# ajparra/iRotAvg

Measured on AMD Instinct MI355X. Metric: IRLS edge-updates/sec (+ iters-to-converge), higher is better.
Workload: dtype f64

## Files before the change

### irotavg_amd/capi.py

```python
import ctypes as C
import os

import numpy as np

_HERE = os.path.dirname(os.path.abspath(__file__))
LIB_PATH = os.path.join(_HERE, "libirotavg_hip.so")

OK = 0
ERR_BAD_ARG, ERR_NOT_SPANNING, ERR_SOLVER, ERR_UNKNOWN_COST = -1, -2, -3, -4
ERR_NOMEM, ERR_HIP, ERR_NO_DEVICE, ERR_NOT_CONVERGED = -5, -6, -7, -8
ERR_UNSUPPORTED = -9

SYMBOLS = [
    "irotavg_default_options", "irotavg_init_mst", "irotavg_make_A", "irotavg_l1ra", "irotavg_irls",
    "irotavg_quat_normalised", "irotavg_graph_create", "irotavg_graph_destroy",
    "irotavg_graph_set_rotations", "irotavg_graph_get_rotations",
    "irotavg_graph_snapshot_rotations", "irotavg_graph_restore_rotations", "irotavg_graph_get_weights",
    "irotavg_graph_set_weights", "irotavg_graph_irls", "irotavg_graph_l1ra",
    "irotavg_graph_quat_normalised", "irotavg_graph_get_stats", "irotavg_graph_reset_stats",
    "irotavg_graph_synchronize", "irotavg_graph_edge_residual", "irotavg_graph_get_residuals",
    "irotavg_graph_ls_solve", "irotavg_graph_update_weights", "irotavg_graph_apply_step",
    "irotavg_graph_l1decode_pd", "irotavg_graph_time_kernel", "irotavg_graph_fingerprint", "irotavg_version",
    "irotavg_device_count", "irotavg_error_string",
    "irotavg_viewgraph_create", "irotavg_viewgraph_destroy", "irotavg_viewgraph_add_view",
# ... 366 lines not shown
        return r

    def ls_solve(self, allow_rc=(), return_rc=False):
        X = np.zeros((self.nu, 3), order="F")
        rc = lib().irotavg_graph_ls_solve(self._h, _d(X), self.nu)
        if rc != OK and rc not in allow_rc:
            raise IrotavgError(rc, "irotavg_graph_ls_solve")
        return (rc, X) if return_rc else X

    def update_weights(self, cost, sigma):
        check(lib().irotavg_graph_update_weights(self._h, cost, sigma), "update_weights")

    def apply_step(self):
        s = C.c_double(0)
        check(lib().irotavg_graph_apply_step(self._h, C.byref(s)), "apply_step")
        return s.value

    def l1decode_pd(self, y, pdmaxiter=2):
        y = np.ascontiguousarray(y, dtype=np.float64)
        assert y.shape == (self.m,)
        x = np.zeros(self.nu)
        stuck = C.c_int(0)
        check(lib().irotavg_graph_l1decode_pd(self._h, _d(y), pdmaxiter, _d(x), C.byref(stuck)),
              "l1decode_pd")
        return x, stuck.value

    def direct_info(self):
        out = (C.c_int64 * 64)()
        k = lib().irotavg_graph_direct_info(self._h, out, 64)
        if k < 0:
            raise IrotavgError(k, "direct_info")
        if out[0] == 0:
            return dict(block=0, levels=[], closures=0, fused_assembly=0, unit_factor=0, unit_factor_solves=0,
                        unit_factor_bytes=0)
        nl = int(out[1])
        return dict(block=int(out[0]), levels=[dict(blocks=int(out[2 + 3 * l]), chunks=int(out[3 + 3 * l]),
                                                    reduced=int(out[4 + 3 * l])) for l in range(nl)],
                    closures=int(out[2 + 3 * nl]), fused_assembly=int(out[3 + 3 * nl]) if k > 3 + 3 * nl else 0,
                    unit_factor=int(out[4 + 3 * nl]) if k > 4 + 3 * nl else 0,
                    unit_factor_solves=int(out[5 + 3 * nl]) if k > 5 + 3 * nl else 0,
                    unit_factor_bytes=int(out[6 + 3 * nl]) if k > 6 + 3 * nl else 0)

    def direct_residual(self):
        out = np.zeros(3)
        check(lib().irotavg_graph_direct_residual(self._h, _d(out)), "direct_residual")
        return out

    def rotation_variance(self, pairs=None, marginals=True, allow_rc=()):
        return _variance_call(lambda *a: lib().irotavg_graph_rotation_variance(self._h, *a), self.n_total, pairs,
                              marginals, allow_rc, "irotavg_graph_rotation_variance")

    def edge_diagnostics(self, edge_var=True, leverage=True, chi2=True, allow_rc=()):
        return _edge_call(lambda *a: lib().irotavg_graph_edge_diagnostics(self._h, *a), self.m, edge_var, leverage,
                          chi2, allow_rc, "irotavg_graph_edge_diagnostics")

    def pose_weights(self, cost, sigma):
        check(lib().irotavg_graph_pose_weights(self._h, int(cost), float(sigma)), "irotavg_graph_pose_weights")

    def fingerprint(self):
        out = (C.c_uint64 * 512)()
        n = lib().irotavg_graph_fingerprint(self._h, out, 512)
        if n < 0:
            raise IrotavgError(n, "fingerprint")
        return [int(out[i]) for i in range(n)]

    FINGERPRINT_TAIL = ("l0_far_entries", "asm_windowed", "asm_l1_fused", "l1_fused", "cg2", "ndense", "ndense_pad",
                        "dense_bw", "mg_dense_max", "mg_kc_x1000", "additive_top")

    def fingerprint_scalars(self):
        fp = self.fingerprint()
        k = len(self.FINGERPRINT_TAIL)
        if not k <= len(fp) < 512:
            raise ValueError("fingerprint truncated: %d words" % len(fp))
        return dict(zip(self.FINGERPRINT_TAIL, fp[-k:]))
# ... 378 lines not shown
```

### irotavg_amd/csrc/bcr.hip

```cpp
#include <atomic>

#include "graph.hpp"
#include "kernels.hpp"
#include "asm0w.hpp"

namespace irh {
constexpr double kBcrGateTolMin = 1e-12;

typedef double v4d __attribute__((ext_vector_type(4)));
typedef double v2d __attribute__((ext_vector_type(2)));
typedef int v2i __attribute__((ext_vector_type(2)));

constexpr int kTopMax = 16, kTopRounds = 6;
struct BcrTopSched {
    int n = 0, nr = 0, last = 0;
    signed char ne[kTopRounds];
    signed char i[kTopRounds][4], a[kTopRounds][4], c[kTopRounds][4];
};

#if defined(__HIP_DEVICE_COMPILE__)
#define IRH_GPTR(T) T __attribute__((address_space(1))) *
#else
#define IRH_GPTR(T) T *
#endif
// ... 1632 lines not shown
        if (NR > 3)
            for (int q = 0; q < nfar; q++) Z[(size_t)row * zstride + zoff + q] = xs[3 + q];
        if (NR == 3 && Qap) acc_ap += step_apply(xs[0], xs[1], xs[2], Qap, row + fap, true);
    };
    if (L0) {
        const int row0 = chunk * 8 * B;
        for (int t = tid; t < kreal * B; t += 256) {
            const int row = row0 + t, blk = t / B;
            if (row < n) put_row(row, bcr_pos(placed, kreal, blk) * B + (t - blk * B));
        }
    } else {
        for (int e = tid; e < 8 * B * NR; e += 256) {
            const int blk = e / (B * NR);
            xl[(size_t)chunk * 8 * B * NR + e] =
                blk < kreal ? (&sX[1][0])[bcr_pos(placed, kreal, blk) * B * NR + (e - blk * B * NR)] : 0.0;
        }
        if (chunk * 8 + 8 > nred && nred < nb)
            for (int t = tid; t < 8 * B; t += 256) {
                const int i = t / B, r = t - i * B, gb = chunk * 8 + i;
                if (gb >= nred && gb < nb) {
                    const int row = (8 * nred + (gb - nred)) * B + r;
                    if (row < n) put_row(row, t);
                }
            }
    }
    if (NR == 3 && Qap) bcr_apply_sum(acc_ap, part_ap, slot0 + chunk);
}

struct BcrBackPlan {
    const double *W[kMaxLevels];
    int nb[kMaxLevels];
    int top, base;
};
constexpr int kBackTopThreads = 512;
template <int B>
__global__ __launch_bounds__(kBackTopThreads) void k_bcr_back_top(BcrBackPlan P, const double *__restrict__ xtop, double *__restrict__ xl,
                                                       double4 *__restrict__ X, int n, int nred,
                                                       double4 *__restrict__ Qap = nullptr, int fap = 0,
                                                       double *__restrict__ part_ap = nullptr, int slot0 = 0,
                                                       int top_all = 0) {
    constexpr int NR = 3;
    typedef BcrDim<B, NR> Dm;
    constexpr int WB = B * Dm::NC, XB = B * NR;
    constexpr int NV = (7 * WB / 2 + kBackTopThreads - 1) / kBackTopThreads;
    __shared__ double sW[7 * WB];
    __shared__ double sX[9][XB];
    __shared__ double sWin[2][16][XB];
    const int tid = threadIdx.x, lane = tid & 63;
    const int wave = __builtin_amdgcn_readfirstlane(tid >> 6);
    const int cbase = blockIdx.x;
    auto range = [&](int L, int &lo, int &hi) {
        lo = hi = cbase;
        for (int l = P.base; l < L; l++) {
            lo = (lo > 0 ? lo - 1 : 0) >> 3;
            hi >>= 3;
        }
    };
    auto wanted = [&](int L, int q) {
        if (L == P.base) return 0x7f;
        int lo, hi, m = 0;
        range(L - 1, lo, hi);
        for (int j = (lo > 0 ? lo - 1 : 0); j <= hi; j++)
            if ((j >> 3) == q && (j & 7) < 7) m |= 1 << (j & 7);
        return bcr_back_mask(m);
    };
    v2d wreg[NV];
    auto request = [&](int L, int q) {
        const int kreal = P.nb[L] - q * 8 < 8 ? P.nb[L] - q * 8 : 8;
        const int nblk = kreal > 7 ? 7 : kreal;
        const int mask = wanted(L, q);
        const v2d *__restrict__ src = reinterpret_cast<const v2d *>(P.W[L] + (size_t)q * 7 * WB);
#pragma unroll
        for (int v = 0; v < NV; v++) {
            const int e = tid + kBackTopThreads * v, blk = e / (WB / 2);
            wreg[v] = (blk < nblk && ((mask >> blk) & 1)) ? __builtin_nontemporal_load(&src[e]) : v2d{0.0, 0.0};
        }
    };
    auto deposit = [&]() {
        v2d *dst = reinterpret_cast<v2d *>(sW);
#pragma unroll
        for (int v = 0; v < NV; v++) {
            const int e = tid + kBackTopThreads * v;
            if (e < 7 * WB / 2) dst[e] = wreg[v];
        }
    };
    double acc_ap = 0.0;
    int L = P.top, lo, hi;
    range(L, lo, hi);
    int q = lo;
    request(L, q);
    while (true) {
        int plo = 0, phi = 0;
        if (L < P.top) range(L + 1, plo, phi);
        const double(*winP)[XB] = sWin[(L + 1) & 1];
        double(*winC)[XB] = sWin[L & 1];
        const int kreal = P.nb[L] - q * 8 < 8 ? P.nb[L] - q * 8 : 8;
        const int mask = wanted(L, q);
        deposit();
        for (int e = tid; e < 7 * XB; e += kBackTopThreads) (&sX[1][0])[e] = 0.0;
        for (int e = tid; e < XB; e += kBackTopThreads) {
            sX[8][e] = L == P.top ? xtop[(top_all ? q * XB : 0) + e] : winP[q - 8 * plo][e];
            sX[0][e] = q == 0 ? 0.0 : L == P.top ? (top_all ? xtop[(q - 1) * XB + e] : 0.0) : winP[q - 1 - 8 * plo][e];
        }
        int Ln = L, qn = q + 1;
        if (qn > hi) {
            Ln = L - 1;
            if (Ln >= P.base) {
                range(Ln, lo, hi);
                qn = lo;
            }
        }
        if (Ln >= P.base) request(Ln, qn);
        __syncthreads();
        bcr_back_rounds<B, NR, kBackTopThreads / 64>(sW, sX, false, kreal, wave, lane, mask);
        if (L > P.base) {
            int clo, chi;
            range(L, clo, chi);
            for (int e = tid; e < 8 * XB; e += kBackTopThreads) {
                const int blk = e / XB;
                winC[(q - clo) * 8 + blk][e - blk * XB] = blk < kreal ? (&sX[1][0])[e] : 0.0;
            }
        } else {
            for (int e = tid; e < 8 * XB; e += kBackTopThreads) {
                const int blk = e / XB;
                xl[(size_t)q * 8 * XB + e] = blk < kreal ? (&sX[1][0])[e] : 0.0;
            }
            if (q * 8 + 8 > nred && nred < P.nb[L])
                for (int t = tid; t < 8 * B; t += kBackTopThreads) {
                    const int i = t / B, r = t - i * B, gb = q * 8 + i;
                    if (gb >= nred && gb < P.nb[L]) {
                        const int row = (8 * nred + (gb - nred)) * B + r;
                        const double *xs = &sX[1][0] + t * NR;
                        if (row < n) {
                            X[row] = double4{xs[0], xs[1], xs[2], 0.0};
                            if (Qap) acc_ap += step_apply(xs[0], xs[1], xs[2], Qap, row + fap, true);
                        }
                    }
                }
        }
        if (Ln < P.base) break;
        __syncthreads();
        L = Ln;
        q = qn;
    }
    if (Qap) bcr_apply_sum(acc_ap, part_ap, slot0 + cbase);
}

struct BcrClPlan {
    const double *W[kMaxLevels], *Dinv[kMaxLevels];
    double *Wrw[kMaxLevels];
    const double *topDinv;
    double *xtop;
};

template <int B, int NWF = 4>
__global__ __launch_bounds__(64 * NWF) void k_bcr_closure_forward(BcrClPlan P, int r, int nslots, const int *__restrict__ off,
                                                              const int4 *__restrict__ steps,
                                                              const int4 *__restrict__ init, double *__restrict__ recR,
                                                              double *__restrict__ recW, double *__restrict__ T,
                                                              const double *__restrict__ slot_init = nullptr,
                                                              const int2 *__restrict__ fin = nullptr,
                                                              const int *__restrict__ gid = nullptr,
                                                              double *__restrict__ dep = nullptr, int world = 0,
                                                              int rank = 0) {
    constexpr int NR = 3, NC = 2 * B + NR, BB = B * B, NCOL = NC + B, NE = B * NCOL;
    constexpr int NLD = (NE + 63) / 64;
    constexpr int KP = B == 24 ? 3 : (NCOL * 4 <= 256 ? 4 : 2), KB = B / KP;
    static_assert(B % KP == 0 && NCOL * KP <= 256, "thread (col, part)");
    extern __shared__ double smem[];
    const int lane = threadIdx.x & 63, wave = __builtin_amdgcn_readfirstlane(threadIdx.x >> 6);
    const int q = blockIdx.x;
    double *stage = smem + (size_t)wave * NE;
    double *spart = smem + (size_t)NWF * NE;
    double *slots = spart + KP * NCOL;
    if (wave == 0) {
        if (slot_init) {
            for (int e = lane; e < nslots * B; e += 64) slots[e] = slot_init[(size_t)q * nslots * B + e];
        } else {
// ... 747 lines not shown
        if (l > 0) L.x.alloc((size_t)L.nch * 8 * B * NR);
        if (nb <= 8 && !g.bcr_shard) {
            S.top16 = false;
            break;
        }
        L.sepD.alloc((size_t)L.nch * B * B);
        L.extD.alloc((size_t)L.nch * B * B);
        L.extG.alloc((size_t)L.nch * B * B);
        L.sepR.alloc((size_t)L.nch * B * NR);
        L.extR.alloc((size_t)L.nch * B * NR);
        if (nb <= 8) break;
        nb = L.nch + (l == 0 ? nraw : 0);
        nch = (nb + 7) / 8;
    }
    if (g.bcr_shard) {
        S.ext0 = g.bcr_ext0;
        S.ghost_extcol.upload(g.bcr_ghost_extcol, g.stream);
        S.remD.alloc((size_t)B * B);
        S.remR.alloc((size_t)B * NR);
        IRH_CHECK(hipStreamSynchronize(g.stream));
    }
    S.xtop.alloc((size_t)B * NR);
    if (S.nfar > 0) bcr_closure_plan(g);
    if (g.bcr_shard && !g.bcr_fix_row.empty()) {
        S.nfix = (int)g.bcr_fix_row.size();
        S.fix_row.upload(g.bcr_fix_row, g.stream);
        S.fix_off.upload(g.bcr_fix_off, g.stream);
        S.fix_e.upload(g.bcr_fix_e, g.stream);
        S.fix_saved.alloc((size_t)S.nfix);
        IRH_CHECK(hipStreamSynchronize(g.stream));
    }
}

template <int B, int NR>
static void bcr_run(Graph &g, int only, int pass, bool open_top = false, int phase = 0, const double *xc_top = nullptr,
                    const double *xext = nullptr) {
    BcrState &S = *g.bcr;
    Level &L0 = g.levels[0];
    hipStream_t st = g.stream;
    const int nl = (int)S.lev.size();
    const int dbg = S.dbg_word >= 0 ? S.dbg_word : g.sw.bcr_dbg;
    long long *stamps = nullptr;
    if (dbg & 64) {
        if (!S.stamps.p) S.stamps.alloc((size_t)S.lev[0].nch * 16);
        stamps = S.stamps.p;
    }
    const int nfar = 0;
    const int *fi = nullptr, *fj = nullptr;
    (void)pass;
    bool fused_up = false;
    if constexpr (NR == 3 && B <= 24) {
        fused_up = nl >= 3 && nl - 1 <= kUpLevels && only < 0 && phase == 0 && !open_top && !g.bcr_shard && S.nfar == 0 &&
                   S.lev[1].nch <= 256 && !(dbg & 64) && !g.bcr_no_fused_up;
        if ((dbg & 128) && !S.stamps.p) S.stamps.alloc((size_t)std::max(S.lev[0].nch * 16, 32 * kUpLevels));
        if (fused_up) fused_up = bcr_up_reserve<B>(g, S.lev[1].nch);
    }
    if (only < 0 && phase != 2) S.up_used = false;
    int uf = 0;
    BcrUnit &U = S.unit;
    if (only < 0 && phase != 2) U.last = 0;
    if constexpr (NR == 3 && (B == 8 || B == 16 || B == 24)) {
        const int req = g.bcr_unit_req;
        if (req && fused_up && S.top16 && dbg == 0 && !g.bcr_guard && !g.bcr_out && !g.sw.bcr_no_unit_factor &&
            (g.bcr_asm_fused || req == 3)) {
            if (!U.lev.empty() && U.epoch != g_unit_epoch.load(std::memory_order_acquire)) U.release();
            uf = U.valid ? 2 : (req == 1 ? 1 : 0);
// ... 167 lines not shown
                }
#undef IRH_BCR_LAUNCH_ASM
            }
        }
        if (asm0) continue;
#define IRH_BCR_LAUNCH(L0_, TOP_)                                                                                   \
    if constexpr (B <= 24) {                                                                                        \
        if (wide)                                                                                                   \
            hipLaunchKernelGGL((k_bcr_reduce<B, NR, L0_, TOP_, 8>), dim3(L.nch), dim3(512), 0, st, IRH_BCR_ARGS);   \
        else                                                                                                        \
            hipLaunchKernelGGL((k_bcr_reduce<B, NR, L0_, TOP_, 4>), dim3(L.nch), dim3(256), 0, st, IRH_BCR_ARGS);   \
    } else {                                                                                                        \
        hipLaunchKernelGGL((k_bcr_reduce<B, NR, L0_, TOP_, 4>), dim3(L.nch), dim3(256), 0, st, IRH_BCR_ARGS);       \
    }
        if (l == 0 && top) {
            IRH_BCR_LAUNCH(true, true)
        } else if (l == 0) {
            IRH_BCR_LAUNCH(true, false)
        } else if (top) {
            IRH_BCR_LAUNCH(false, true)
        } else {
            IRH_BCR_LAUNCH(false, false)
        }
#undef IRH_BCR_LAUNCH
#undef IRH_BCR_ARGS
    }
    double4 *Xout = g.bcr_out ? g.bcr_out : g.X.p + g.ng;
    bool fused_back = false;
    const int ltop = S.top16 ? nl - 2 : nl - 1;
    if constexpr (NR == 3) fused_back = ltop >= 1 && !g.bcr_shard && !open_top;
    const bool apply = NR == 3 && g.bcr_apply && only < 0 && phase == 0 && (fused_back || (S.top16 && nl == 2)) && !g.bcr_out &&
                       g.ng == 0;
    g.bcr_applied = apply;
    for (int l = ltop; l >= 0 && phase != 1 && !uf_up_only; l--) {
        if (only >= 0 && only != 100 + l) continue;
        BcrLevel &L = S.lev[l];
        if constexpr (NR == 3) {
            if (fused_back && l >= 1) {
                if (l > 1) continue;
                BcrBackPlan P;
                for (int k = 0; k < nl; k++) {
                    P.W[k] = uf && k + 1 < nl ? U.lev[(size_t)k].Wu.p : S.lev[k].W.p;
                    P.nb[k] = S.lev[k].nb;
                }
                P.top = ltop;
                P.base = 1;
                hipLaunchKernelGGL((k_bcr_back_top<B>), dim3(L.nch), dim3(kBackTopThreads), 0, st, P,
                                   S.top16 ? S.lev[nl - 1].x.p : S.xtop.p, L.x.p, Xout, L0.n, L.nred,
                                   apply ? g.Q.p : (double4 *)nullptr, g.f, g.part_score.p, S.lev[0].nch, (int)S.top16);
                continue;
            }
        }
        const double *xc = l == nl - 1 ? (open_top ? xc_top : S.xtop.p) : S.lev[l + 1].x.p;
        if (l == 0)
            hipLaunchKernelGGL((k_bcr_back<B, NR, true>), dim3(L.nch), dim3(256), 0, st, L.nb, L.nred, L0.n,
                               uf ? U.lev[0].Wu.p : L.W.p, xc,
                               (double *)nullptr, Xout, (double *)nullptr, 0, 0, nfar, xext, (int)g.bcr_shard,
                               apply ? g.Q.p : (double4 *)nullptr, g.f, g.part_score.p, 0);
        else
            hipLaunchKernelGGL((k_bcr_back<B, NR, false>), dim3(L.nch), dim3(256), 0, st, L.nb, L.nred, L0.n, L.W.p, xc,
                               L.x.p, Xout, (double *)nullptr, 0, 0, nfar, xext, (int)g.bcr_shard);
    }
}

template <int B>
static void bcr_launch_forward(hipStream_t st, const BcrClPlan &P, int r, int nslots, const int *off, const int4 *steps,
                               const int4 *init, double *recR, double *recW, double *T, const double *slot_init,
                               const int2 *fin, const int *gid, double *dep, int world, int rank);

template <int B>
static void bcr_run_all(Graph &g, int only) {
    BcrState &S = *g.bcr;
    if (S.nfar == 0 || only >= 0) {
        bcr_run<B, 3>(g, only, 0);
        return;
    }
    hipStream_t st = g.stream;
    const int r = S.nfar, npad = S.cl_npad, nl = (int)S.lev.size();
    if (!S.dead_clean) IRH_CHECK(hipMemsetAsync(S.dead.p, 0, sizeof(int), st));
// ... 361 lines not shown
    T.co_elim.upload(elim, st);
    T.xbuf.alloc(T.x_doubles());
    T.Dinv.alloc((size_t)7 * B * B);
    T.topDinv.alloc((size_t)B * B);
    T.recR.alloc((size_t)r * nst * B);
    T.recW.alloc((size_t)r * nst * B);
    T.Ttop.alloc((size_t)r * 3);
    T.lam.alloc((size_t)T.npad * 3);
    T.dead.alloc(1);
    IRH_CHECK(hipMemsetAsync(T.topDinv.p, 0, sizeof(double) * (size_t)B * B, st));
    IRH_CHECK(hipMemsetAsync(T.xbuf.p, 0, sizeof(double) * T.x_doubles(), st));
    IRH_CHECK(hipStreamSynchronize(st));
}
#define IRH_BCR_DISPATCH(fn, ...)              \
    switch (g.bcr_B) {                         \
    case 8: fn<8>(__VA_ARGS__); break;         \
    case 16: fn<16>(__VA_ARGS__); break;       \
    case 24: fn<24>(__VA_ARGS__); break;       \
    default: fn<32>(__VA_ARGS__); break;       \
    }
void bcr_shard_reduce(Graph &g, BcrTop &T, int rank) {
    bcr_alloc(g);
    IRH_BCR_DISPATCH(bcr_shard_reduce_t, g, T, rank)
}
void bcr_top_solve(Graph &g, BcrTop &T) { IRH_BCR_DISPATCH(bcr_top_solve_t, g, T) }
void bcr_shard_back(Graph &g, BcrTop &T, int rank) {
    IRH_BCR_DISPATCH(bcr_shard_back_t, g, T, rank)
    g.stats.direct_solves += 1;
}
void bcr_shard_closures_forward(Graph &g, BcrTop &T, int rank) { IRH_BCR_DISPATCH(bcr_shard_closures_forward_t, g, T, rank) }
void bcr_top_solve_closures(Graph &g, BcrTop &T) { IRH_BCR_DISPATCH(bcr_top_solve_closures_t, g, T) }
void bcr_shard_closures_correct(Graph &g, BcrTop &T) { IRH_BCR_DISPATCH(bcr_shard_closures_correct_t, g, T) }

int bcr_solve(Graph &g, int only) {
    if (!g.bcr_B) return IROTAVG_ERR_BAD_ARG;
    bcr_alloc(g);
    switch (g.bcr_B) {
    case 8: bcr_run_all<8>(g, only); break;
    case 12: bcr_run_all<12>(g, only); break;
    case 16: bcr_run_all<16>(g, only); break;
    case 20: bcr_run_all<20>(g, only); break;
    case 24: bcr_run_all<24>(g, only); break;
    case 28: bcr_run_all<28>(g, only); break;
    case 32: bcr_run_all<32>(g, only); break;
    default: return IROTAVG_ERR_BAD_ARG;
    }
    if (only < 0) g.stats.direct_solves += 1;
    return IROTAVG_OK;
}

__global__ __launch_bounds__(256) void k_bcr_residual(int n, const int *__restrict__ sl_off, const int *__restrict__ col,
                                                       const double *__restrict__ val, const double *__restrict__ diag,
                                                       const double4 *__restrict__ rhs, const double4 *__restrict__ X,
                                                       double *__restrict__ part) {
    const int row = blockIdx.x * 256 + threadIdx.x;
    double r0 = 0.0, r1 = 0.0, r2 = 0.0, b0 = 0.0, b1 = 0.0, b2 = 0.0;
    if (row < n) {
        const int sl = row >> 6, ln = row & 63;
        const int o0 = sl_off[sl], w = sl_off[sl + 1] - o0;
        const v2i *__restrict__ cp = reinterpret_cast<const v2i *>(col) + (size_t)(o0 / 2) * 64 + ln;
        const v2d *__restrict__ vp = reinterpret_cast<const v2d *>(val) + (size_t)(o0 / 2) * 64 + ln;
        const double4 x = X[row], bb = rhs[row];
        const double d = diag[row];
        double s0 = d * x.x, s1 = d * x.y, s2 = d * x.z;
        for (int q = 0; q < w / 2; q++) {
            const v2i cc = cp[(size_t)q * 64];
// ... 42 lines not shown
    double rr[3] = {0, 0, 0}, bb[3] = {0, 0, 0};
    for (int b = 0; b < grid; b++)
        for (int c = 0; c < 3; c++) {
            rr[c] += h[(size_t)b * 8 + c];
            bb[c] += h[(size_t)b * 8 + 4 + c];
        }
    for (int c = 0; c < 3; c++) {
        relres[c] = bb[c] > 0.0 ? std::sqrt(rr[c] / bb[c]) : (rr[c] > 0.0 ? HUGE_VAL : 0.0);
        g.stats.last_relres[c] = relres[c];
    }
    return IROTAVG_OK;
}

int bcr_info(Graph &g, int64_t *out, int cap) {
    int k = 0;
    auto put = [&](int64_t v) {
        if (k < cap) out[k++] = v;
    };
    put(g.bcr_B);
    if (!g.bcr_B) return k;
    bcr_alloc(g);
    put((int64_t)g.bcr->lev.size());
    for (const BcrLevel &L : g.bcr->lev) {
        put(L.nb);
        put(L.nch);
        put(L.nred);
    }
    put(g.bcr->nfar);
    put(g.bcr_asm_fused_last ? 1 : 0);
    const bool stored = bcr_unit_valid(g);
    put(stored ? 1 : 0);
    put(g.bcr->unit.solves);
    put(stored ? g.bcr->unit.bytes : 0);
    return k;
}

int bcr_stamps_up(Graph &g, double *out) {
    if (!g.bcr_B) return IROTAVG_ERR_BAD_ARG;
    bcr_alloc(g);
    BcrState &S = *g.bcr;
    struct DbgScope {
        BcrState &S;
        ~DbgScope() { S.dbg_word = -1; }
    } dbg_scope{S};
    S.dbg_word = 128 + 256 * g.sw.bcr_stamp_chunk;
    const size_t cnt = (size_t)std::max(S.lev[0].nch * 16, 32 * kUpLevels);
    if (!S.stamps.p) S.stamps.alloc(cnt);
    IRH_CHECK(hipMemsetAsync(S.stamps.p, 0, sizeof(long long) * cnt, g.stream));
    const int rc = bcr_solve(g, -1);
    S.dbg_word = -1;
    if (rc != IROTAVG_OK) return rc;
    long long h[32 * kUpLevels];
    IRH_CHECK(hipMemcpyAsync(h, S.stamps.p, sizeof(h), hipMemcpyDeviceToHost, g.stream));
    IRH_CHECK(hipStreamSynchronize(g.stream));
    bcr_up_release(g);
    for (int k = 0; k < 32 * kUpLevels; k++) out[k] = !h[k] ? -1.0 : (k & 31) >= 20 ? (double)h[k] : (double)(h[k] - h[16]);
    return S.up_used ? IROTAVG_OK : IROTAVG_ERR_BAD_ARG;
}

int bcr_stamps(Graph &g, int level, int chunk, double *out) {
    if (!g.bcr_B) return IROTAVG_ERR_BAD_ARG;
    bcr_alloc(g);
    BcrState &S = *g.bcr;
    if (level < 0 || level >= (int)S.lev.size() || chunk < 0 || chunk >= S.lev[level].nch) return IROTAVG_ERR_BAD_ARG;
    struct DbgScope {
        BcrState &S;
// ... 562 lines not shown
```

### irotavg_amd/csrc/graph.hpp

```cpp
#pragma once
#include <functional>
#include <memory>

#include "common.hpp"
#include "hostwait.hpp"

namespace irh {

struct Graph;
void bcr_up_release(Graph &g) noexcept;
struct BcrState;
struct BcrDeleter {
    void operator()(BcrState *p) const;
};

struct Graph {
    int64_t m = 0, n_total = 0, mpad = 0;
    int f = 0, nu = 0, ng = 0, no = 0;
    irotavg_options opt{};
    Switches sw;
    hipStream_t stream = nullptr;
    int device = 0;

    DevBuf<int> ei, ej;
// ... 59 lines not shown

    DevBuf<double> pd;
    DevBuf<double> pdn;
    DevBuf<double> pd_part;
    bool pd_ready = false;
    const double *pd_rhs_src = nullptr;
    bool pd_rhs_done = false;
    std::vector<std::unique_ptr<Graph>> l1_clones;
    bool is_clone = false;

    double *hpin = nullptr;
    double *h_part() { return hpin; }
    double *h_scal() { return hpin + 4 * kMaxParts; }
    int *h_flags() { return reinterpret_cast<int *>(hpin + 4 * kMaxParts + SC_COUNT); }
    int *h_seq() { return reinterpret_cast<int *>(hpin + 8192); }
    int pub_seq = 0;
    hipEvent_t ev_in = nullptr, ev_out = nullptr;
    ~Graph() {
        bcr_up_release(*this);
        if (ev_in) (void)hipEventDestroy(ev_in);
        if (ev_out) (void)hipEventDestroy(ev_out);
        if (hpin) PinPool::get().give(hpin);
    }
    Graph() = default;
    Graph(const Graph &) = delete;
    Graph &operator=(const Graph &) = delete;

    int bcr_B = 0, band0 = -1;
    bool bcr_apply = false, bcr_applied = false;
    int bcr_up_held = 0;
    bool pool_headroom = false;
    bool bcr_no_fused_up = false;
    bool bcr_asm_fused = false, bcr_asm_fused_last = false;
    int bcr_unit_req = 0;
    std::unique_ptr<BcrState, BcrDeleter> bcr;
    std::vector<int> bcr_far_i, bcr_far_j, bcr_far_e;
    const double *bcr_wsrc = nullptr;
    int bcr_wsquare = 0;
    bool bcr_guard = false;
    bool bcr_last_guarded = false;
    double4 *bcr_out = nullptr;
    bool bcr_shard = false;
    int bcr_ext0 = 0;
    std::vector<int> bcr_ghost_extcol;
    std::vector<int> bcr_far_gid;
    std::vector<uint8_t> bcr_far_own;
    std::vector<int> bcr_fix_row, bcr_fix_off, bcr_fix_e;

    double last_score_sum = 0.0;
    double irls_settle = -1.0;
    int force_np = 0;
    irotavg_stats stats{};
};

struct PrecInfo {
    int np_rz = 0, np_rz2 = 0;
};

struct BuildTail {
    int nlev = 1;
    int agg[kMaxLevels] = {0};
    int dense_bw = 0;
    bool l1_window_ok = false;
    bool l1_band8 = false;
};
struct HierPlan {
// ... 136 lines not shown
    const int32_t *prow;
    double *pair_var;
    int nc;
    const int32_t *crow;
    const double *cq;
    double *angle, *cand_var, *cand_chi2;
    double s2;
};
int wincov_query(WinCov &wc, WinCovQuery &q);
struct WinCovPlan;
struct WinCovArrays {
    const int32_t *I;
    const double *QQ;
    long long qq_rs, qq_cs;
    const double *Q;
    long long q_rs, q_cs;
    const double *weights;
    double *var;
    const int32_t *pairs;
    double *pair_var;
    double *edge_var, *leverage, *chi2;
    bool gate = false;
    const int32_t *cand = nullptr;
    const double *cand_QQ = nullptr;
    long long cq_rs = 0, cq_cs = 0;
    double *angle = nullptr, *cand_var = nullptr, *cand_chi2 = nullptr;
};
int wincov_batch_dev(const WinCovPlan &plan, int device, const WinCovArrays &A, double sigma, double *scale ,
                     int32_t *results , hipStream_t stream);
void launch_pose_weights(Graph &g, int cost, double sigma);
void candidate_angles(Graph &g, int64_t n, const double *q12, double *angle);
void bcr_plan(Graph &g, const int32_t *I);
void bcr_plan_dev(Graph &g, const DevEdgeSrc &src);
int bcr_solve(Graph &g, int only = -1);
int bcr_levels(Graph &g);
int bcr_info(Graph &g, int64_t *out, int cap);
int bcr_residual(Graph &g, double *relres);
int bcr_closures(Graph &g);
constexpr double kClosureRepairAccept = 1e-8;
bool bcr_band_part_anchored(int64_t m, int f, int64_t nu, int B, const int32_t *I);
int bcr_apply_slots(Graph &g);
void bcr_gate(Graph &g, double *flags_copy = nullptr);
const int *bcr_gate_skip_word(Graph &g);
void dense_invert_spd(Graph &g, double *A, int npad);
int bcr_stamps(Graph &g, int level, int chunk, double *out);
int bcr_stamps_up(Graph &g, double *out);
int bcr_rhs_products(int B, const double *Dinv, const double *P, const double *Q, const double *R, int hasP, int hasQ,
                     double *WR, double *Ra, double *Rc);
int bcr_block_products(int B, int wpe, const double *Dinv, const double *P, const double *Q, const double *R, int hasP,
                       int hasQ, double *Dc, double *Da, double *W, double *fill);
bool bcr_up_failed(Graph &g);
void bcr_unit_commit(Graph &g, bool finite);
int bcr_unit_last(Graph &g);
bool bcr_unit_valid(Graph &g);
void bcr_unit_trim() noexcept;
const int *bcr_fail_word(Graph &g);
struct BcrTop {
    int B = 0, world = 0;
    DevBuf<double> buf;
    DevBuf<double> rec;
    size_t record_doubles() const { return 3 * (size_t)B * B + 2 * (size_t)B * 3; }
    DevBuf<double> W, x, xtop;
    size_t n_doubles() const { return (size_t)world * (3 * (size_t)B * B + 2 * (size_t)B * 3); }
    int r = 0, npad = 0, nst = 0;
    DevBuf<double> xbuf, Dinv, topDinv, recR, recW, Ttop, lam;
    DevBuf<int> dead, cl_off, cl_owner, co_off, co_rec;
// ... 61 lines not shown
```

### irotavg_amd/csrc/kernels.hpp

```cpp
#pragma once
#include "common.hpp"

namespace irh {

struct LevelView {
    int n, nsl, agg;
    const int *sl_off, *sl_near, *col;
    const double *val, *diag, *idg;
};

inline LevelView view_of(const Level &L) {
    return LevelView{L.n, L.nsl, L.agg, L.sl_off.p, L.sl_near.p, L.col.p, L.val.p, L.diag.p, L.idg.p};
}

__device__ __forceinline__ double wave_sum(double v) {
#pragma unroll
    for (int o = 32; o > 0; o >>= 1) v += __shfl_down(v, o, 64);
    return v;
}
__device__ __forceinline__ double wave_min(double v) {
#pragma unroll
    for (int o = 32; o > 0; o >>= 1) v = fmin(v, __shfl_down(v, o, 64));
    return v;
}
// ... 333 lines not shown
        return 1.0 / sqrt(1.0 + e2 / (t * t));
    }
    case IROTAVG_FAIR:
        return 1.0 / sqrt(1.0 + sqrt(e2) / (1.400 * sigma));
    case IROTAVG_LOGISTIC: {
        const double e = sqrt(e2) / (1.205 * sigma);
        return e < 0.0001 ? 1.0 : sqrt(tanh(e) / e);
    }
    case IROTAVG_TALWAR: {
        const double t = 2.795 * sigma;
        return e2 < t * t ? 1.0001 : 0.0;
    }
    default: {
        const double t = 2.985 * sigma;
        double w = exp(-.5 * e2 / (t * t));
        return w < 0.0001 ? 0.0001 : w;
    }
    }
}

__device__ __forceinline__ double4 step_quat(double x0, double x1, double x2, double &th) {
    th = sqrt(x0 * x0 + x1 * x1 + x2 * x2);
    double sn, cs;
    sincos(th / 2.0, &sn, &cs);
    const double coef = sn / th;
    double4 w = make_double4(x0 * coef, x1 * coef, x2 * coef, cs);
    if (!isfinite(w.x)) w.x = 0.0;
    if (!isfinite(w.y)) w.y = 0.0;
    if (!isfinite(w.z)) w.z = 0.0;
    if (!isfinite(w.w)) w.w = 0.0;
    return w;
}

__device__ __forceinline__ double step_apply(double x0, double x1, double x2, double4 *__restrict__ Q, int idx, bool write) {
    double th;
    const double4 w = step_quat(x0, x1, x2, th);
    const double4 q = qmul(Q[idx], w);
    if (write && isfinite(th)) Q[idx] = q;
    return th;
}

}
```

### irotavg_amd/csrc/solver.hip

```cpp
#include <cstring>

#include "graph.hpp"
#include "kernels.hpp"
#include "asm0w.hpp"

namespace irh {


__global__ __launch_bounds__(256) void k_edge_residual(long long mpad, const int *__restrict__ ei,
                                                       const int *__restrict__ ej,
                                                       const double *__restrict__ qq,
                                                       const double4 *__restrict__ Q,
                                                       double *__restrict__ er, double *__restrict__ ones) {
    const long long k = 2ll * ((long long)blockIdx.x * blockDim.x + threadIdx.x);
    if (k >= mpad) return;
    if (ones) *reinterpret_cast<double2 *>(ones + k) = make_double2(1.0, 1.0);
    const int2 ii = *reinterpret_cast<const int2 *>(ei + k);
    const int2 jj = *reinterpret_cast<const int2 *>(ej + k);
    const double2 qx = *reinterpret_cast<const double2 *>(qq + k);
    const double2 qy = *reinterpret_cast<const double2 *>(qq + mpad + k);
    const double2 qz = *reinterpret_cast<const double2 *>(qq + 2 * mpad + k);
    const double2 qw = *reinterpret_cast<const double2 *>(qq + 3 * mpad + k);
    const double4 qi0 = Q[ii.x], qj0 = Q[jj.x], qi1 = Q[ii.y], qj1 = Q[jj.y];
    double2 rx, ry, rz;
// ... 2156 lines not shown
            break;
        case 5: (void)precondition(g, 0, -1.0); break;
        case 8: {
            Level &L0 = g.levels[0];
            hipLaunchKernelGGL((k_pspmv_dot<false, false>), dim3(grid_for_rows(L0)), dim3(kRowBlock), 0, g.stream,
                               view_of(L0), __builtin_ctz((unsigned)L0.agg), g.scal.p, 0, g.part_rz.p, 1,
                               g.part_rz2.p, 1, L0.b.p, g.levels[1].y.p, g.opt.mg_omega, g.opt.mg_kc, g.P.p,
                               g.P2.p, g.AP.p, g.part_pq.p, g.flags.p);
            break;
        }
        case 9: cg2_time_once(g, 0); break;
        case 10: cg2_time_once(g, 1); break;
        case 11: launch_weights_then_residual(g, IROTAVG_GEMAN_MCCLURE, 5 * IRH_PI / 180.0, nullptr, true); break;
        case 12: launch_pose_weights(g, IROTAVG_GEMAN_MCCLURE, 5 * IRH_PI / 180.0); break;
        case 6:
            hipLaunchKernelGGL(k_apply_step, dim3(grid_for_elems(g.nu)), dim3(kRowBlock), 0, g.stream,
                               g.nu, g.f, g.ng, g.X.p, g.Q.p, g.part_score.p, 0, (const int *)nullptr);
            break;
        default:
            if (which == 19) (void)bcr_solve(g);
            else if (which == 17 || which == 18) {
                g.bcr_unit_req = which == 17 ? 2 : 3;
                g.bcr_asm_fused = which == 17;
                g.bcr_wsrc = g.dw.p;
                g.bcr_wsquare = 1;
                (void)bcr_solve(g);
                g.bcr_unit_req = 0;
                g.bcr_asm_fused = false;
                unit_served = unit_served && bcr_unit_last(g) == 2;
                bcr_unit_commit(g, false);
            }
            else if (which >= 20 && which < 40) (void)bcr_solve(g, which - 20);
            else if (which >= 40 && which < 60) (void)bcr_solve(g, 100 + which - 40);
            break;
        }
    };
    if (which == 17 || which == 18) {
        if (!g.bcr_B || !bcr_unit_valid(g)) return IROTAVG_ERR_BAD_ARG;
    } else if (which >= 19 && which < 60) {
        if (!g.bcr_B) return IROTAVG_ERR_BAD_ARG;
        const int nl = bcr_levels(g);
        if ((which >= 20 && which < 40 && which - 20 >= nl) || (which >= 40 && which - 40 >= nl)) return IROTAVG_ERR_BAD_ARG;
    } else if (which < 1 || which > 12) return IROTAVG_ERR_BAD_ARG;
    if ((which == 9 || which == 10) && !g.cg2) return IROTAVG_ERR_BAD_ARG;
    if (which == 8 && !(g.additive_top && g.levels.size() > 1 && g.ng == 0 && g.l0_far_entries == 0 &&
                        g.opt.no_fused_pspmv != 1))
        return IROTAVG_ERR_BAD_ARG;
    IRH_CHECK(hipMemsetAsync(g.flags.p, 0, sizeof(int) * FL_COUNT, g.stream));
    DevBuf<double> keep_dw, keep_er;
    if (which == 11 || which == 12) {
        keep_dw.alloc((size_t)g.mpad);
        keep_er.alloc((size_t)3 * g.mpad);
        IRH_CHECK(hipMemcpyAsync(keep_dw.p, g.dw.p, sizeof(double) * (size_t)g.mpad, hipMemcpyDeviceToDevice, g.stream));
        IRH_CHECK(hipMemcpyAsync(keep_er.p, g.er.p, sizeof(double) * 3 * (size_t)g.mpad, hipMemcpyDeviceToDevice, g.stream));
    }
    once();
    IRH_CHECK(hipEventRecord(e0, g.stream));
    for (int r = 0; r < reps; r++) once();
    IRH_CHECK(hipEventRecord(e1, g.stream));
    if (which == 11 || which == 12) {
        IRH_CHECK(hipMemcpyAsync(g.dw.p, keep_dw.p, sizeof(double) * (size_t)g.mpad, hipMemcpyDeviceToDevice, g.stream));
        IRH_CHECK(hipMemcpyAsync(g.er.p, keep_er.p, sizeof(double) * 3 * (size_t)g.mpad, hipMemcpyDeviceToDevice, g.stream));
        IRH_CHECK(hipStreamSynchronize(g.stream));
    }
    IRH_CHECK(hipEventSynchronize(e1));
    bcr_up_release(g);
    float t = 0.f;
    IRH_CHECK(hipEventElapsedTime(&t, e0, e1));
    *ms = (double)t / std::max(reps, 1);
    (void)hipEventDestroy(e0);
// ... 7 lines not shown
```

### irotavg_amd/csrc/switches.hpp

```cpp
#pragma once
#include <algorithm>
#include <cstdlib>
#include <tuple>

namespace irh {

struct Switches {
    bool has_band_direct = false;
    int band_direct = 0;
    int host_build = -1;
    int upload_threads = 4;
    bool asm_classic = false, no_small_tuning = false;
    bool no_dense_refine = false, no_band_inverse = false, pcg_trace = false;
    int cg2_giveup = 0;
    bool no_settle = false, no_fused_cl = false;
    int inexact = -1;
    bool bcr_no_mixed = false, bcr_no_top16 = false, bcr_fake_up_fail = false, bcr_fake_give_up = false;
    bool bcr_no_closures = false, bcr_s_tiles = false, bcr_no_fused_asm = false, bcr_no_unit_factor = false;
    int bcr_up_cap = 1024;
    int bcr_dbg = 0, bcr_stamp_chunk = 0;
    bool dist_no_closures = false, dist_halo_p2p = false;
    bool no_resident = false, window_stamps = false;
    long resident_min_edges = 20000;
    bool build_timing = false, rotavg_timing = false;
};

inline Switches read_switches() {
    Switches s;
    auto set = [](const char *name) { return std::getenv(name) != nullptr; };
    auto num = [](const char *name, int unset) {
        const char *e = std::getenv(name);
        return e ? std::atoi(e) : unset;
    };
    s.has_band_direct = set("IROTAVG_BAND_DIRECT");
    s.band_direct = num("IROTAVG_BAND_DIRECT", 0);
    s.host_build = set("IROTAVG_HOST_BUILD") ? (num("IROTAVG_HOST_BUILD", 0) != 0 ? 1 : 0) : -1;
    s.upload_threads = std::min(4, std::max(0, num("IROTAVG_UPLOAD_THREADS", 4)));
    s.asm_classic = set("IROTAVG_ASM_CLASSIC");
    s.no_small_tuning = set("IROTAVG_NO_SMALL_TUNING");
    s.no_dense_refine = set("IROTAVG_NO_DENSE_REFINE");
    s.no_band_inverse = set("IROTAVG_NO_BAND_INVERSE");
    s.pcg_trace = set("IROTAVG_PCG_TRACE");
    s.cg2_giveup = set("IROTAVG_CG2_GIVEUP") ? std::max(1, num("IROTAVG_CG2_GIVEUP", 0)) : 0;
    s.no_settle = set("IROTAVG_NO_SETTLE");
    s.no_fused_cl = set("IROTAVG_NO_FUSED_CL");
    s.inexact = set("IROTAVG_INEXACT") ? (num("IROTAVG_INEXACT", 0) != 0 ? 1 : 0) : -1;
    s.bcr_no_mixed = set("IROTAVG_BCR_NO_MIXED");
    s.bcr_no_top16 = set("IROTAVG_BCR_NO_TOP16");
    s.bcr_fake_up_fail = set("IROTAVG_BCR_FAKE_UP_FAIL");
    s.bcr_fake_give_up = set("IROTAVG_BCR_FAKE_GIVE_UP");
    s.bcr_no_closures = set("IROTAVG_BCR_NO_CLOSURES");
    s.bcr_s_tiles = set("IROTAVG_BCR_S_TILES");
    s.bcr_no_fused_asm = set("IROTAVG_BCR_NO_FUSED_ASM");
    s.bcr_no_unit_factor = set("IROTAVG_BCR_NO_UNIT_FACTOR");
    s.bcr_up_cap = num("IROTAVG_BCR_UP_CAP", 1024);
    s.bcr_dbg = num("IROTAVG_BCR_DBG", 0);
    s.bcr_stamp_chunk = num("IROTAVG_BCR_STAMP_CHUNK", 0);
    s.dist_no_closures = set("IROTAVG_DIST_NO_CLOSURES");
    s.dist_halo_p2p = set("IROTAVG_DIST_HALO_P2P");
    s.no_resident = set("IROTAVG_NO_RESIDENT");
    s.window_stamps = set("IROTAVG_WINDOW_STAMPS");
    if (const char *e = std::getenv("IROTAVG_RESIDENT_MIN_EDGES")) s.resident_min_edges = std::atol(e);
    s.build_timing = set("IROTAVG_BUILD_TIMING");
    s.rotavg_timing = set("IROTAVG_ROTAVG_TIMING");
    return s;
}

inline bool operator==(const Switches &a, const Switches &b) {
    auto t = [](const Switches &s) {
        return std::make_tuple(
            s.has_band_direct, s.band_direct, s.host_build, s.upload_threads, s.asm_classic, s.no_small_tuning,
            s.no_dense_refine, s.no_band_inverse, s.pcg_trace, s.cg2_giveup, s.no_settle, s.no_fused_cl, s.inexact,
            s.bcr_no_mixed, s.bcr_no_top16, s.bcr_fake_up_fail, s.bcr_fake_give_up, s.bcr_no_closures, s.bcr_s_tiles,
            s.bcr_no_fused_asm, s.bcr_no_unit_factor, s.bcr_up_cap, s.bcr_dbg, s.bcr_stamp_chunk, s.dist_no_closures, s.dist_halo_p2p, s.no_resident, s.window_stamps,
            s.resident_min_edges, s.build_timing, s.rotavg_timing);
    };
    return t(a) == t(b);
}

inline const char *env_pool_limit_mb() { return std::getenv("IROTAVG_POOL_LIMIT_MB"); }
inline bool env_pin_default() { return std::getenv("IROTAVG_PIN_DEFAULT") != nullptr; }
inline bool env_no_poll() { return std::getenv("IROTAVG_NO_POLL") != nullptr || env_pin_default(); }
inline bool env_oneshot_cache() {
    const char *e = std::getenv("IROTAVG_ONESHOT_CACHE");
    return !(e && std::atoi(e) == 0);
}
inline int env_build_threads() {
    const char *e = std::getenv("IROTAVG_BUILD_THREADS");
    return e ? std::min(16, std::max(1, std::atoi(e))) : 0;
}

}
```

Before: 8.589 billion.

## Fuse BCR back-substitution into a single launch covering all levels

Adds a k_bcr_back_all kernel in which each level-0 chunk block walks the whole back-substitution from the top level down to level 0 on its own. It also handles one raw level-1 block per workgroup and applies the rotation step, which replaces the previous two-launch scheme (back_top plus a level-0 pass). The goal is to remove a kernel launch and the round trip of intermediate level solutions through global memory. In exchange, blocks redundantly recompute upper-level windows. The path is gated on occupancy (grid must fit co-resident), top16, at least 3 levels and no sharding, and can be disabled with an env switch.

```diff
diff --git a/irotavg_amd/capi.py b/irotavg_amd/capi.py
--- a/irotavg_amd/capi.py
+++ b/irotavg_amd/capi.py
@@ -422,14 +422,15 @@
             raise IrotavgError(k, "direct_info")
         if out[0] == 0:
             return dict(block=0, levels=[], closures=0, fused_assembly=0, unit_factor=0, unit_factor_solves=0,
-                        unit_factor_bytes=0)
+                        unit_factor_bytes=0, fused_back=0)
         nl = int(out[1])
         return dict(block=int(out[0]), levels=[dict(blocks=int(out[2 + 3 * l]), chunks=int(out[3 + 3 * l]),
                                                     reduced=int(out[4 + 3 * l])) for l in range(nl)],
                     closures=int(out[2 + 3 * nl]), fused_assembly=int(out[3 + 3 * nl]) if k > 3 + 3 * nl else 0,
                     unit_factor=int(out[4 + 3 * nl]) if k > 4 + 3 * nl else 0,
                     unit_factor_solves=int(out[5 + 3 * nl]) if k > 5 + 3 * nl else 0,
-                    unit_factor_bytes=int(out[6 + 3 * nl]) if k > 6 + 3 * nl else 0)
+                    unit_factor_bytes=int(out[6 + 3 * nl]) if k > 6 + 3 * nl else 0,
+                    fused_back=int(out[7 + 3 * nl]) if k > 7 + 3 * nl else 0)
 
     def direct_residual(self):
         out = np.zeros(3)
diff --git a/irotavg_amd/csrc/bcr.hip b/irotavg_amd/csrc/bcr.hip
--- a/irotavg_amd/csrc/bcr.hip
+++ b/irotavg_amd/csrc/bcr.hip
@@ -1688,6 +1688,49 @@
     int nb[kMaxLevels];
     int top, base;
 };
+template <int B, int NT>
+struct BcrBackWalk {
+    static constexpr int WB = B * BcrDim<B, 3>::NC;
+    static constexpr int NV = (7 * WB / 2 + NT - 1) / NT;
+    const BcrBackPlan &P;
+    int base, cbase, basemask;
+    __device__ __forceinline__ void range(int L, int &lo, int &hi) const {
+        lo = hi = cbase;
+        for (int l = base; l < L; l++) {
+            lo = (lo > 0 ? lo - 1 : 0) >> 3;
+            hi >>= 3;
+        }
+    }
+    __device__ __forceinline__ int wanted(int L, int q) const {
+        if (L == base) return basemask;
+        int lo, hi, m = 0;
+        range(L - 1, lo, hi);
+        for (int j = (lo > 0 ? lo - 1 : 0); j <= hi; j++)
+            if ((j >> 3) == q && (j & 7) < 7) m |= 1 << (j & 7);
+        return bcr_back_mask(m);
+    }
+    __device__ __forceinline__ void request(v2d (&wreg)[NV], int L, int q) const {
+        const int tid = threadIdx.x;
+        const int kreal = P.nb[L] - q * 8 < 8 ? P.nb[L] - q * 8 : 8;
+        const int nblk = kreal > 7 ? 7 : kreal;
+        const int mask = wanted(L, q);
+        const v2d *__restrict__ src = reinterpret_cast<const v2d *>(P.W[L] + (size_t)q * 7 * WB);
+#pragma unroll
+        for (int v = 0; v < NV; v++) {
+            const int e = tid + NT * v, blk = e / (WB / 2);
+            wreg[v] = (blk < nblk && ((mask >> blk) & 1)) ? __builtin_nontemporal_load(&src[e]) : v2d{0.0, 0.0};
+        }
+    }
+    __device__ __forceinline__ static void deposit(const v2d (&wreg)[NV], double *sW) {
+        const int tid = threadIdx.x;
+        v2d *dst = reinterpret_cast<v2d *>(sW);
+#pragma unroll
+        for (int v = 0; v < NV; v++) {
+            const int e = tid + NT * v;
+            if (e < 7 * WB / 2) dst[e] = wreg[v];
+        }
+    }
+};
 constexpr int kBackTopThreads = 512;
 template <int B>
 __global__ __launch_bounds__(kBackTopThreads) void k_bcr_back_top(BcrBackPlan P, const double *__restrict__ xtop, double *__restrict__ xl,
@@ -1697,49 +1740,20 @@
                                                        int top_all = 0) {
     constexpr int NR = 3;
     typedef BcrDim<B, NR> Dm;
+    typedef BcrBackWalk<B, kBackTopThreads> Walk;
     constexpr int WB = B * Dm::NC, XB = B * NR;
-    constexpr int NV = (7 * WB / 2 + kBackTopThreads - 1) / kBackTopThreads;
     __shared__ double sW[7 * WB];
     __shared__ double sX[9][XB];
     __shared__ double sWin[2][16][XB];
     const int tid = threadIdx.x, lane = tid & 63;
     const int wave = __builtin_amdgcn_readfirstlane(tid >> 6);
     const int cbase = blockIdx.x;
-    auto range = [&](int L, int &lo, int &hi) {
-        lo = hi = cbase;
-        for (int l = P.base; l < L; l++) {
-            lo = (lo > 0 ? lo - 1 : 0) >> 3;
-            hi >>= 3;
-        }
-    };
-    auto wanted = [&](int L, int q) {
-        if (L == P.base) return 0x7f;
-        int lo, hi, m = 0;
-        range(L - 1, lo, hi);
-        for (int j = (lo > 0 ? lo - 1 : 0); j <= hi; j++)
-            if ((j >> 3) == q && (j & 7) < 7) m |= 1 << (j & 7);
-        return bcr_back_mask(m);
-    };
-    v2d wreg[NV];
-    auto request = [&](int L, int q) {
-        const int kreal = P.nb[L] - q * 8 < 8 ? P.nb[L] - q * 8 : 8;
-        const int nblk = kreal > 7 ? 7 : kreal;
-        const int mask = wanted(L, q);
-        const v2d *__restrict__ src = reinterpret_cast<const v2d *>(P.W[L] + (size_t)q * 7 * WB);
-#pragma unroll
-        for (int v = 0; v < NV; v++) {
-            const int e = tid + kBackTopThreads * v, blk = e / (WB / 2);
-            wreg[v] = (blk < nblk && ((mask >> blk) & 1)) ? __builtin_nontemporal_load(&src[e]) : v2d{0.0, 0.0};
-        }
-    };
-    auto deposit = [&]() {
-        v2d *dst = reinterpret_cast<v2d *>(sW);
-#pragma unroll
-        for (int v = 0; v < NV; v++) {
-            const int e = tid + kBackTopThreads * v;
-            if (e < 7 * WB / 2) dst[e] = wreg[v];
-        }
-    };
+    const Walk walk{P, P.base, cbase, 0x7f};
+    auto range = [&](int L, int &lo, int &hi) { walk.range(L, lo, hi); };
+    auto wanted = [&](int L, int q) { return walk.wanted(L, q); };
+    v2d wreg[Walk::NV];
+    auto request = [&](int L, int q) { walk.request(wreg, L, q); };
+    auto deposit = [&]() { Walk::deposit(wreg, sW); };
     double acc_ap = 0.0;
     int L = P.top, lo, hi;
     range(L, lo, hi);
@@ -1800,6 +1814,123 @@
         q = qn;
     }
     if (Qap) bcr_apply_sum(acc_ap, part_ap, slot0 + cbase);
+}
+
+constexpr int kBackAllThreads = 256;
+template <int B>
+__global__ __launch_bounds__(kBackAllThreads, 2) void k_bcr_back_all(BcrBackPlan Parg, const double *__restrict__ xtop,
+                                                                     double4 *__restrict__ X, int n, int nred, int nraw,
+                                                                     double4 *__restrict__ Qap, int fap,
+                                                                     double *__restrict__ part_ap, int nzero) {
+    constexpr int NR = 3, NT = kBackAllThreads;
+    typedef BcrDim<B, NR> Dm;
+    typedef BcrBackWalk<B, NT> Walk;
+    constexpr int WB = B * Dm::NC, XB = B * NR;
+    static_assert(3 * XB <= NT && 8 * B <= NT, "a thread per entry of the window and per row of a chunk");
+    __shared__ double sW[7 * WB];
+    __shared__ double sX[9][XB];
+    __shared__ double sWin[2][3][XB];
+    __shared__ BcrBackPlan P;
+    const int tid = threadIdx.x, lane = tid & 63;
+    const int wave = __builtin_amdgcn_readfirstlane(tid >> 6);
+    if (tid < kMaxLevels) {
+        P.W[tid] = Parg.W[tid];
+        P.nb[tid] = Parg.nb[tid];
+    }
+    if (tid == 0) P.top = Parg.top;
+    __syncthreads();
+    const int c = blockIdx.x;
+    const int rr = (int)gridDim.x - 1 - c;
+    const bool raw = rr < nraw;
+    const int rblk = nred + rr, rpos = rblk & 7;
+    const Walk own{P, 0, c, 0x7f};
+    const Walk rwk{P, 1, rblk >> 3, rpos < 7 ? bcr_back_mask(1 << rpos) : 0};
+    auto top_window = [&](const Walk &w) {
+        int lo, hi;
+        w.range(P.top, lo, hi);
+        const int blk = tid / XB, j = (lo > 0 ? lo - 1 : 0) + blk;
+        return tid < 3 * XB && j <= hi ? xtop[(size_t)j * XB + (tid - blk * XB)] : 0.0;
+    };
+    const double xw_own = top_window(own), xw_raw = raw ? top_window(rwk) : 0.0;
+    v2d wreg[Walk::NV];
+    {
+        int lo, hi;
+        own.range(P.top, lo, hi);
+        own.request(wreg, P.top, lo);
+    }
+    const int kreal0 = P.nb[0] - c * 8 < 8 ? P.nb[0] - c * 8 : 8;
+    const int row_own = c * 8 * B + tid, row_raw = (8 * nred + rr) * B + tid;
+    const bool has_own = tid < kreal0 * B && row_own < n, has_raw = raw && tid < B && row_raw < n;
+    double4 q_own = double4{0.0, 0.0, 0.0, 0.0}, q_raw = q_own;
+    if (Qap && has_own) q_own = Qap[row_own + fap];
+    if (Qap && has_raw) q_raw = Qap[row_raw + fap];
+    double xs_own[NR] = {0.0, 0.0, 0.0}, xs_raw[NR] = {0.0, 0.0, 0.0};
+    for (int pass = 0; pass < (raw ? 2 : 1); pass++) {
+        const Walk w = pass == 0 ? own : rwk;
+        if (tid < 3 * XB) (&sWin[(P.top + 1) & 1][0][0])[tid] = pass == 0 ? xw_own : xw_raw;
+        __syncthreads();
+        int L = P.top, lo, hi;
+        w.range(L, lo, hi);
+        int q = lo;
+        while (true) {
+            const int jlo = lo > 0 ? lo - 1 : 0;
+            const double(*winP)[XB] = sWin[(L + 1) & 1];
+            double(*winC)[XB] = sWin[L & 1];
+            const int kreal = P.nb[L] - q * 8 < 8 ? P.nb[L] - q * 8 : 8;
+            const int mask = w.wanted(L, q);
+            Walk::deposit(wreg, sW);
+            for (int e = tid; e < 7 * XB; e += NT) (&sX[1][0])[e] = 0.0;
+            for (int e = tid; e < XB; e += NT) {
+                sX[8][e] = winP[q - jlo][e];
+                sX[0][e] = q == 0 ? 0.0 : winP[q - 1 - jlo][e];
+            }
+            int Ln = L, qn = q + 1;
+            if (qn > hi) {
+                Ln = L - 1;
+                if (Ln >= w.base) {
+                    w.range(Ln, lo, hi);
+                    qn = lo;
+                }
+            }
+            if (Ln >= w.base) {
+                w.request(wreg, Ln, qn);
+            } else if (pass == 0 && raw) {
+                int rlo, rhi;
+                rwk.range(P.top, rlo, rhi);
+                rwk.request(wreg, P.top, rlo);
+            }
+            __syncthreads();
+            bcr_back_rounds<B, NR, NT / 64>(sW, sX, false, kreal, wave, lane, mask);
+            if (L > w.base) {
+                int l2, h2;
+                w.range(L - 1, l2, h2);
+                const int blk = tid / XB, j = (l2 > 0 ? l2 - 1 : 0) + blk, pos = j & 7;
+                if (tid < 3 * XB && j <= h2 && (j >> 3) == q)
+                    winC[blk][tid - blk * XB] = pos < kreal ? sX[pos + 1][tid - blk * XB] : 0.0;
+            } else if (pass == 0) {
+                if (has_own)
+                    for (int k = 0; k < NR; k++) xs_own[k] = (&sX[1][0])[tid * NR + k];
+            } else {
+                if (has_raw)
+                    for (int k = 0; k < NR; k++) xs_raw[k] = sX[1 + rpos][tid * NR + k];
+            }
+            if (Ln < w.base) break;
+            __syncthreads();
+            L = Ln;
+            q = qn;
+        }
+    }
+    double acc_ap = 0.0;
+    auto put_row = [&](int row, const double *xs, const double4 &q0) {
+        X[row] = double4{xs[0], xs[1], xs[2], 0.0};
+        if (Qap) acc_ap += step_apply_to(xs[0], xs[1], xs[2], q0, Qap, row + fap, true);
+    };
+    if (has_own) put_row(row_own, xs_own, q_own);
+    if (has_raw) put_row(row_raw, xs_raw, q_raw);
+    if (Qap) {
+        bcr_apply_sum(acc_ap, part_ap, c);
+        if (tid == 0 && c < nzero) part_ap[gridDim.x + c] = 0.0;
+    }
 }
 
 struct BcrClPlan {
@@ -2613,6 +2744,27 @@
     }
 }
 
+template <int B>
+static bool bcr_back_all_ok(Graph &g) {
+    static std::atomic<int> cap[16];
+    const BcrState &S = *g.bcr;
+    const int nl = (int)S.lev.size();
+    if (!S.top16 || nl < 3 || S.nfar != 0 || g.bcr_shard || g.ng != 0 || g.sw.bcr_two_launch_back) return false;
+    const int nch0 = S.lev[0].nch;
+    if (S.lev[1].nb - S.lev[1].nred > nch0 || S.lev[1].nch > nch0) return false;
+    const int d = g.device & 15;
+    int c = cap[d].load(std::memory_order_relaxed);
+    if (c == 0) {
+        int per_cu = 0, cus = 0;
+        if (hipOccupancyMaxActiveBlocksPerMultiprocessor(&per_cu, k_bcr_back_all<B>, kBackAllThreads, 0) != hipSuccess) per_cu = 0;
+        if (hipDeviceGetAttribute(&cus, hipDeviceAttributeMultiprocessorCount, g.device) != hipSuccess) cus = 0;
+        (void)hipGetLastError();
+        c = per_cu >= 2 && cus > 0 ? per_cu * cus : -1;
+        cap[d].store(c, std::memory_order_relaxed);
+    }
+    return c > 0 && nch0 <= c;
+}
+
 template <int B, int NR>
 static void bcr_run(Graph &g, int only, int pass, bool open_top = false, int phase = 0, const double *xc_top = nullptr,
                     const double *xext = nullptr) {
@@ -2846,19 +2998,37 @@
     const bool apply = NR == 3 && g.bcr_apply && only < 0 && phase == 0 && (fused_back || (S.top16 && nl == 2)) && !g.bcr_out &&
                        g.ng == 0;
     g.bcr_applied = apply;
+    auto back_plan = [&](int base) {
+        BcrBackPlan P;
+        for (int k = 0; k < nl; k++) {
+            P.W[k] = uf && k + 1 < nl ? U.lev[(size_t)k].Wu.p : S.lev[k].W.p;
+            P.nb[k] = S.lev[k].nb;
+        }
+        P.top = ltop;
+        P.base = base;
+        return P;
+    };
+    bool back_all = false;
+    if constexpr (NR == 3 && (B == 8 || B == 16 || B == 24))
+        back_all = bcr_back_all_ok<B>(g) && !g.bcr_guard && !g.bcr_out && dbg == 0 && phase == 0 && !open_top &&
+                   ((fused_up && apply) || only == 200);
+    if (only < 0 && phase != 1) g.bcr_back_all_last = back_all;
+    if constexpr (NR == 3 && (B == 8 || B == 16 || B == 24)) {
+        if (back_all) {
+            const BcrLevel &L1 = S.lev[1];
+            hipLaunchKernelGGL((k_bcr_back_all<B>), dim3(S.lev[0].nch), dim3(kBackAllThreads), 0, st, back_plan(0),
+                               S.lev[nl - 1].x.p, Xout, L0.n, L1.nred, L1.nb - L1.nred, apply ? g.Q.p : (double4 *)nullptr,
+                               g.f, g.part_score.p, L1.nch);
+            return;
+        }
+    }
     for (int l = ltop; l >= 0 && phase != 1 && !uf_up_only; l--) {
         if (only >= 0 && only != 100 + l) continue;
         BcrLevel &L = S.lev[l];
         if constexpr (NR == 3) {
             if (fused_back && l >= 1) {
                 if (l > 1) continue;
-                BcrBackPlan P;
-                for (int k = 0; k < nl; k++) {
-                    P.W[k] = uf && k + 1 < nl ? U.lev[(size_t)k].Wu.p : S.lev[k].W.p;
-                    P.nb[k] = S.lev[k].nb;
-                }
-                P.top = ltop;
-                P.base = 1;
+                const BcrBackPlan P = back_plan(1);
                 hipLaunchKernelGGL((k_bcr_back_top<B>), dim3(L.nch), dim3(kBackTopThreads), 0, st, P,
                                    S.top16 ? S.lev[nl - 1].x.p : S.xtop.p, L.x.p, Xout, L0.n, L.nred,
                                    apply ? g.Q.p : (double4 *)nullptr, g.f, g.part_score.p, S.lev[0].nch, (int)S.top16);
@@ -3286,6 +3456,17 @@
 void bcr_top_solve_closures(Graph &g, BcrTop &T) { IRH_BCR_DISPATCH(bcr_top_solve_closures_t, g, T) }
 void bcr_shard_closures_correct(Graph &g, BcrTop &T) { IRH_BCR_DISPATCH(bcr_shard_closures_correct_t, g, T) }
 
+bool bcr_back_all_handle(Graph &g) {
+    if (!g.bcr_B) return false;
+    bcr_alloc(g);
+    switch (g.bcr_B) {
+    case 8: return bcr_back_all_ok<8>(g);
+    case 16: return bcr_back_all_ok<16>(g);
+    case 24: return bcr_back_all_ok<24>(g);
+    default: return false;
+    }
+}
+
 int bcr_solve(Graph &g, int only) {
     if (!g.bcr_B) return IROTAVG_ERR_BAD_ARG;
     bcr_alloc(g);
@@ -3394,6 +3575,7 @@
     put(stored ? 1 : 0);
     put(g.bcr->unit.solves);
     put(stored ? g.bcr->unit.bytes : 0);
+    put(g.bcr_back_all_last ? 1 : 0);
     return k;
 }
 
diff --git a/irotavg_amd/csrc/graph.hpp b/irotavg_amd/csrc/graph.hpp
--- a/irotavg_amd/csrc/graph.hpp
+++ b/irotavg_amd/csrc/graph.hpp
@@ -115,6 +115,7 @@
     bool pool_headroom = false;
     bool bcr_no_fused_up = false;
     bool bcr_asm_fused = false, bcr_asm_fused_last = false;
+    bool bcr_back_all_last = false;
     int bcr_unit_req = 0;
     std::unique_ptr<BcrState, BcrDeleter> bcr;
     std::vector<int> bcr_far_i, bcr_far_j, bcr_far_e;
@@ -317,6 +318,7 @@
 void candidate_angles(Graph &g, int64_t n, const double *q12, double *angle);
 void bcr_plan(Graph &g, const int32_t *I);
 void bcr_plan_dev(Graph &g, const DevEdgeSrc &src);
+bool bcr_back_all_handle(Graph &g);
 int bcr_solve(Graph &g, int only = -1);
 int bcr_levels(Graph &g);
 int bcr_info(Graph &g, int64_t *out, int cap);
diff --git a/irotavg_amd/csrc/kernels.hpp b/irotavg_amd/csrc/kernels.hpp
--- a/irotavg_amd/csrc/kernels.hpp
+++ b/irotavg_amd/csrc/kernels.hpp
@@ -389,12 +389,16 @@
     return w;
 }
 
-__device__ __forceinline__ double step_apply(double x0, double x1, double x2, double4 *__restrict__ Q, int idx, bool write) {
+__device__ __forceinline__ double step_apply_to(double x0, double x1, double x2, const double4 &q0, double4 *__restrict__ Q,
+                                                int idx, bool write) {
     double th;
     const double4 w = step_quat(x0, x1, x2, th);
-    const double4 q = qmul(Q[idx], w);
+    const double4 q = qmul(q0, w);
     if (write && isfinite(th)) Q[idx] = q;
     return th;
 }
-
-}
+__device__ __forceinline__ double step_apply(double x0, double x1, double x2, double4 *__restrict__ Q, int idx, bool write) {
+    return step_apply_to(x0, x1, x2, Q[idx], Q, idx, write);
+}
+
+}
diff --git a/irotavg_amd/csrc/solver.hip b/irotavg_amd/csrc/solver.hip
--- a/irotavg_amd/csrc/solver.hip
+++ b/irotavg_amd/csrc/solver.hip
@@ -2212,10 +2212,13 @@
             }
             else if (which >= 20 && which < 40) (void)bcr_solve(g, which - 20);
             else if (which >= 40 && which < 60) (void)bcr_solve(g, 100 + which - 40);
+            else if (which == 16) (void)bcr_solve(g, 200);
             break;
         }
     };
-    if (which == 17 || which == 18) {
+    if (which == 16) {
+        if (!bcr_back_all_handle(g)) return IROTAVG_ERR_BAD_ARG;
+    } else if (which == 17 || which == 18) {
         if (!g.bcr_B || !bcr_unit_valid(g)) return IROTAVG_ERR_BAD_ARG;
     } else if (which >= 19 && which < 60) {
         if (!g.bcr_B) return IROTAVG_ERR_BAD_ARG;
diff --git a/irotavg_amd/csrc/switches.hpp b/irotavg_amd/csrc/switches.hpp
--- a/irotavg_amd/csrc/switches.hpp
+++ b/irotavg_amd/csrc/switches.hpp
@@ -17,6 +17,7 @@
     int inexact = -1;
     bool bcr_no_mixed = false, bcr_no_top16 = false, bcr_fake_up_fail = false, bcr_fake_give_up = false;
     bool bcr_no_closures = false, bcr_s_tiles = false, bcr_no_fused_asm = false, bcr_no_unit_factor = false;
+    bool bcr_two_launch_back = false;
     int bcr_up_cap = 1024;
     int bcr_dbg = 0, bcr_stamp_chunk = 0;
     bool dist_no_closures = false, dist_halo_p2p = false;
@@ -53,6 +54,7 @@
     s.bcr_s_tiles = set("IROTAVG_BCR_S_TILES");
     s.bcr_no_fused_asm = set("IROTAVG_BCR_NO_FUSED_ASM");
     s.bcr_no_unit_factor = set("IROTAVG_BCR_NO_UNIT_FACTOR");
+    s.bcr_two_launch_back = set("IROTAVG_BCR_TWO_LAUNCH_BACK");
     s.bcr_up_cap = num("IROTAVG_BCR_UP_CAP", 1024);
     s.bcr_dbg = num("IROTAVG_BCR_DBG", 0);
     s.bcr_stamp_chunk = num("IROTAVG_BCR_STAMP_CHUNK", 0);
@@ -72,7 +74,7 @@
             s.has_band_direct, s.band_direct, s.host_build, s.upload_threads, s.asm_classic, s.no_small_tuning,
             s.no_dense_refine, s.no_band_inverse, s.pcg_trace, s.cg2_giveup, s.no_settle, s.no_fused_cl, s.inexact,
             s.bcr_no_mixed, s.bcr_no_top16, s.bcr_fake_up_fail, s.bcr_fake_give_up, s.bcr_no_closures, s.bcr_s_tiles,
-            s.bcr_no_fused_asm, s.bcr_no_unit_factor, s.bcr_up_cap, s.bcr_dbg, s.bcr_stamp_chunk, s.dist_no_closures, s.dist_halo_p2p, s.no_resident, s.window_stamps,
+            s.bcr_no_fused_asm, s.bcr_no_unit_factor, s.bcr_two_launch_back, s.bcr_up_cap, s.bcr_dbg, s.bcr_stamp_chunk, s.dist_no_closures, s.dist_halo_p2p, s.no_resident, s.window_stamps,
             s.resident_min_edges, s.build_timing, s.rotavg_timing);
     };
     return t(a) == t(b);
```

Result: slower. 8.171 billion (-4.9%).
